# sczhou/CodeFormer

Hardware: NVIDIA H100
Metric: faces_per_sec_512x512_batch32 (higher is better)
Workload: dtype f32 (split-fp16 operands on tensor cores, fp32 accumulate)

## Files before the change

codeformer_b200/csrc/simt_kernels.cu:

```cuda
#include <cuda_fp16.h>
#include <cuda_runtime.h>

#include <atomic>
#include <math.h>
#include <stdint.h>

#include "kernels.cuh"

namespace cfb {

__device__ __forceinline__ float silu_f(float x) { return x / (1.f + expf(-x)); }
__device__ __forceinline__ float gelu_f(float x) { return 0.5f * x * (1.f + erff(x * 0.70710678118654752440f)); }
__device__ __forceinline__ float lrelu_f(float x) { return x > 0.f ? x : 0.2f * x; }

constexpr int CF_BM = 128;
constexpr int CF_BK = 16;
constexpr int CF_APITCH = CF_BM + 4;

template <int BN>
__global__ void __launch_bounds__(256) conv_f32_kernel(ConvArgs a) {
  constexpr int TN = BN / 16;
  __shared__ __align__(16) float As[2][CF_BK][CF_APITCH];
  __shared__ __align__(16) float Bs[2][CF_BK][BN];

  const int t = threadIdx.x;
  const int64_t M = (int64_t)a.N * a.Ho * a.Wo;
  const int64_t m0 = (int64_t)blockIdx.x * CF_BM;
  const int n0 = blockIdx.y * BN;
  const int taps = a.ksize * a.ksize;
  const int kchunks = a.Cin / CF_BK;
  const int nk = taps * kchunks;

  const int arow = t >> 1;
  const int akq = (t & 1) * 8;
  const int64_t am = m0 + arow;
  const bool arow_ok = am < M;
  int an = 0, aoy = 0, aox = 0;
  if (arow_ok) {
    an = (int)(am / ((int64_t)a.Ho * a.Wo));
    int rem = (int)(am - (int64_t)an * a.Ho * a.Wo);
    aoy = rem / a.Wo;
    aox = rem - aoy * a.Wo;
  }
  const float* in_n = a.in + (int64_t)an * a.H * a.W * a.Cin;
  const float* sc_n = a.in_scale ? a.in_scale + (int64_t)an * a.Cin : nullptr;
  const float* sh_n = a.in_shift ? a.in_shift + (int64_t)an * a.Cin : nullptr;

  constexpr int BV = (CF_BK * BN / 4) / 256;
  const int bcol = (BN == 128) ? (t & 31) * 4 : (t & 15) * 4;
  const int brow0 = (BN == 128) ? (t >> 5) : (t >> 4);

  float4 ra[2], rb[BV];

  auto load_global = [&](int it) {
    const int tap = it / kchunks;
    const int c0 = (it - tap * kchunks) * CF_BK;
    int r = 0, s = 0;
    if (a.ksize == 3) { r = tap / 3; s = tap - r * 3; }
    bool ok = arow_ok;
    int iy, ix;
    if (a.mode == CONV_DOWN) {
      iy = aoy * 2 + r; ix = aox * 2 + s;
      ok = ok && iy < a.H && ix < a.W;
    } else if (a.mode == CONV_UP) {
      iy = aoy + r - 1; ix = aox + s - 1;
      ok = ok && iy >= 0 && ix >= 0 && iy < 2 * a.H && ix < 2 * a.W;
      iy >>= 1; ix >>= 1;
    } else {
      const int p = a.ksize >> 1;
      iy = aoy + r - p; ix = aox + s - p;
      ok = ok && iy >= 0 && ix >= 0 && iy < a.H && ix < a.W;
    }
    if (ok) {
      const float* p = in_n + ((int64_t)iy * a.W + ix) * a.Cin + c0 + akq;
      ra[0] = __ldg(reinterpret_cast<const float4*>(p));
      ra[1] = __ldg(reinterpret_cast<const float4*>(p + 4));
      if (sc_n) {
        const float4 s0 = __ldg(reinterpret_cast<const float4*>(sc_n + c0 + akq));
        const float4 s1 = __ldg(reinterpret_cast<const float4*>(sc_n + c0 + akq + 4));
        const float4 h0 = __ldg(reinterpret_cast<const float4*>(sh_n + c0 + akq));
        const float4 h1 = __ldg(reinterpret_cast<const float4*>(sh_n + c0 + akq + 4));
        ra[0].x = fmaf(ra[0].x, s0.x, h0.x); ra[0].y = fmaf(ra[0].y, s0.y, h0.y);
        ra[0].z = fmaf(ra[0].z, s0.z, h0.z); ra[0].w = fmaf(ra[0].w, s0.w, h0.w);
        ra[1].x = fmaf(ra[1].x, s1.x, h1.x); ra[1].y = fmaf(ra[1].y, s1.y, h1.y);
        ra[1].z = fmaf(ra[1].z, s1.z, h1.z); ra[1].w = fmaf(ra[1].w, s1.w, h1.w);
      }
      if (a.in_act == IN_SILU) {
        ra[0].x = silu_f(ra[0].x); ra[0].y = silu_f(ra[0].y); ra[0].z = silu_f(ra[0].z); ra[0].w = silu_f(ra[0].w);
        ra[1].x = silu_f(ra[1].x); ra[1].y = silu_f(ra[1].y); ra[1].z = silu_f(ra[1].z); ra[1].w = silu_f(ra[1].w);
      }
    } else {
      ra[0] = make_float4(0.f, 0.f, 0.f, 0.f);
      ra[1] = ra[0];
    }
    const float* wb = a.wgt_f32 + ((int64_t)tap * a.Cin + c0) * a.Cout + n0 + bcol;
#pragma unroll
    for (int i = 0; i < BV; ++i) {
      const int kr = brow0 + i * 8;
      rb[i] = __ldg(reinterpret_cast<const float4*>(wb + (int64_t)kr * a.Cout));
    }
  };
  auto store_smem = [&](int buf) {
    As[buf][akq + 0][arow] = ra[0].x; As[buf][akq + 1][arow] = ra[0].y;
    As[buf][akq + 2][arow] = ra[0].z; As[buf][akq + 3][arow] = ra[0].w;
    As[buf][akq + 4][arow] = ra[1].x; As[buf][akq + 5][arow] = ra[1].y;
    As[buf][akq + 6][arow] = ra[1].z; As[buf][akq + 7][arow] = ra[1].w;
#pragma unroll
    for (int i = 0; i < BV; ++i) {
      const int kr = brow0 + i * 8;
      *reinterpret_cast<float4*>(&Bs[buf][kr][bcol]) = rb[i];
    }
  };

  const int ty = t >> 4, tx = t & 15;
  float acc[8][TN];
#pragma unroll
  for (int i = 0; i < 8; ++i)
#pragma unroll
    for (int j = 0; j < TN; ++j) acc[i][j] = 0.f;

  load_global(0);
  store_smem(0);
  __syncthreads();
  int buf = 0;
  for (int it = 0; it < nk; ++it) {
    if (it + 1 < nk) load_global(it + 1);
#pragma unroll
    for (int k = 0; k < CF_BK; ++k) {
      const float4 a0 = *reinterpret_cast<const float4*>(&As[buf][k][ty * 4]);
      const float4 a1 = *reinterpret_cast<const float4*>(&As[buf][k][64 + ty * 4]);
      const float av[8] = {a0.x, a0.y, a0.z, a0.w, a1.x, a1.y, a1.z, a1.w};
      float bv[TN];
      {
        const float4 b0 = *reinterpret_cast<const float4*>(&Bs[buf][k][tx * 4]);
        bv[0] = b0.x; bv[1] = b0.y; bv[2] = b0.z; bv[3] = b0.w;
        if (TN == 8) {
          const float4 b1 = *reinterpret_cast<const float4*>(&Bs[buf][k][(BN / 2) + tx * 4]);
          bv[TN - 4] = b1.x; bv[TN - 3] = b1.y; bv[TN - 2] = b1.z; bv[TN - 1] = b1.w;
        }
      }
#pragma unroll
      for (int i = 0; i < 8; ++i)
#pragma unroll
        for (int j = 0; j < TN; ++j) acc[i][j] = fmaf(av[i], bv[j], acc[i][j]);
    }
    if (it + 1 < nk) store_smem(buf ^ 1);
    __syncthreads();
    buf ^= 1;
  }

#pragma unroll
  for (int i = 0; i < 8; ++i) {
    const int64_t m = m0 + ((i < 4) ? (ty * 4 + i) : (64 + ty * 4 + (i - 4)));
    if (m >= M) continue;
#pragma unroll
    for (int h = 0; h < TN / 4; ++h) {
      const int col = n0 + h * (BN / 2) + tx * 4;
      float4 v = make_float4(acc[i][h * 4 + 0], acc[i][h * 4 + 1], acc[i][h * 4 + 2], acc[i][h * 4 + 3]);
      if (a.bias) {
        const float4 b = __ldg(reinterpret_cast<const float4*>(a.bias + col));
        v.x += b.x; v.y += b.y; v.z += b.z; v.w += b.w;
      }
      const int64_t off = m * a.Cout + col;
      if (a.residual) {
        const float4 r = __ldg(reinterpret_cast<const float4*>(a.residual + off));
        v.x += r.x; v.y += r.y; v.z += r.z; v.w += r.w;
      }
      if (a.out_act == OUT_LRELU) {
        v.x = lrelu_f(v.x); v.y = lrelu_f(v.y); v.z = lrelu_f(v.z); v.w = lrelu_f(v.w);
      } else if (a.out_act == OUT_GELU) {
        v.x = gelu_f(v.x); v.y = gelu_f(v.y); v.z = gelu_f(v.z); v.w = gelu_f(v.w);
      }
      if (a.sft_dec) {
        const float4 d = __ldg(reinterpret_cast<const float4*>(a.sft_dec + off));
        const float4 s = __ldg(reinterpret_cast<const float4*>(a.sft_scale + off));
        v.x = d.x + a.sft_w * (d.x * s.x + v.x); v.y = d.y + a.sft_w * (d.y * s.y + v.y);
        v.z = d.z + a.sft_w * (d.z * s.z + v.z); v.w = d.w + a.sft_w * (d.w * s.w + v.w);
      }
      *reinterpret_cast<float4*>(a.out + off) = v;
    }
  }
}

int conv_f32(const ConvArgs& a, cudaStream_t st) {
  CFB_REQUIRE(a.Cin % CF_BK == 0, "conv_f32: Cin must be a multiple of 16");
  CFB_REQUIRE(a.Cout % 64 == 0, "conv_f32: Cout must be a multiple of 64");
  CFB_REQUIRE(a.ksize == 1 || a.ksize == 3, "conv_f32: kernel size must be 1 or 3");
  CFB_REQUIRE(a.wgt_f32 && a.in && a.out, "conv_f32: null tensor");
  const int64_t M = (int64_t)a.N * a.Ho * a.Wo;
  if (M == 0) return 0;
  const unsigned gx = (unsigned)((M + CF_BM - 1) / CF_BM);
  if (a.Cout % 128 == 0) {
    conv_f32_kernel<128><<<dim3(gx, a.Cout / 128), 256, 0, st>>>(a);
  } else {
    conv_f32_kernel<64><<<dim3(gx, a.Cout / 64), 256, 0, st>>>(a);
  }
  CFB_LAUNCH_CHECK();
  return 0;
}

__device__ __forceinline__ float u8_to_model_input(int u) {
  const float t = (float)((double)u / 255.0);
  return __fdiv_rn(__fsub_rn(t, 0.5f), 0.5f);
}
__device__ __forceinline__ unsigned model_output_to_u8(float v) {
  float t = fminf(fmaxf(v, -1.f), 1.f);
  t = __fdiv_rn(__fadd_rn(t, 1.f), 2.f);
  return (unsigned)rintf(__fmul_rn(t, 255.f));
}

template <int COUT, bool U8>
__global__ void __launch_bounds__(256) conv_first_kernel(const float* __restrict__ x, const float* __restrict__ wgt,
                                                         const float* __restrict__ bias, float* __restrict__ out,
                                                         int N, int H, int W, float* __restrict__ gn_part) {
  __shared__ __align__(16) float ws[27 * COUT];
  __shared__ float bs[COUT];
  __shared__ float lut[U8 ? 256 : 1];
  if constexpr (U8) lut[threadIdx.x] = u8_to_model_input(threadIdx.x);
  pdl_launch_dependents();
  pdl_wait();
  for (int i = threadIdx.x; i < 27 * COUT; i += 256) ws[i] = wgt[i];
  for (int i = threadIdx.x; i < COUT; i += 256) bs[i] = bias ? bias[i] : 0.f;
  __syncthreads();
  constexpr int CPT = COUT / 4;
  const int64_t HW = (int64_t)H * W;
  const int64_t quad = (int64_t)blockIdx.x * 64 + (threadIdx.x >> 2);
  const int cg = threadIdx.x & 3;
  const int64_t pix0 = quad * 4;
  if (pix0 >= (int64_t)N * HW) return;
  const int n = (int)(pix0 / HW);
  const int rem = (int)(pix0 - (int64_t)n * HW);
  const int y = rem / W, x0 = rem - y * W;
  float acc[4][CPT];
#pragma unroll
  for (int p = 0; p < 4; ++p)
#pragma unroll
    for (int j = 0; j < CPT; ++j) acc[p][j] = bs[cg * CPT + j];
#pragma unroll
  for (int r = 0; r < 3; ++r) {
    const int iy = y + r - 1;
    const bool rowok = iy >= 0 && iy < H;
#pragma unroll
    for (int c = 0; c < 3; ++c) {
      float v[6];
      if constexpr (U8) {
        const unsigned char* rp8 = reinterpret_cast<const unsigned char*>(x) + ((int64_t)n * HW + (int64_t)iy * W) * 3 + (2 - c);
#pragma unroll
        for (int q = 0; q < 6; ++q) {
          const int ix = x0 + q - 1;
          v[q] = (rowok && ix >= 0 && ix < W) ? lut[__ldg(rp8 + ix * 3)] : 0.f;
        }
      } else {
        const float* rp = x + ((int64_t)n * 3 + c) * HW + (int64_t)iy * W;
#pragma unroll
        for (int q = 0; q < 6; ++q) {
          const int ix = x0 + q - 1;
          v[q] = (rowok && ix >= 0 && ix < W) ? __ldg(rp + ix) : 0.f;
        }
      }
#pragma unroll
      for (int s = 0; s < 3; ++s) {
        const float* wr = ws + ((r * 3 + s) * 3 + c) * COUT + cg * CPT;
#pragma unroll
        for (int j = 0; j < CPT; j += 4) {
          const float4 w4 = *reinterpret_cast<const float4*>(wr + j);
#pragma unroll
          for (int p = 0; p < 4; ++p) {
            acc[p][j] = fmaf(v[p + s], w4.x, acc[p][j]); acc[p][j + 1] = fmaf(v[p + s], w4.y, acc[p][j + 1]);
            acc[p][j + 2] = fmaf(v[p + s], w4.z, acc[p][j + 2]); acc[p][j + 3] = fmaf(v[p + s], w4.w, acc[p][j + 3]);
          }
        }
      }
    }
  }
#pragma unroll
  for (int p = 0; p < 4; ++p) {
    float* o = out + (pix0 + p) * COUT + cg * CPT;
#pragma unroll
    for (int j = 0; j < CPT; j += 4) *reinterpret_cast<float4*>(o + j) = make_float4(acc[p][j], acc[p][j + 1], acc[p][j + 2], acc[p][j + 3]);
  }
  if (gn_part != nullptr) {
    static_assert(COUT == 64, "GroupNorm partials: two channels per group");
    float gs[CPT / 2], gq[CPT / 2];
#pragma unroll
    for (int g = 0; g < CPT / 2; ++g) {
      float a = 0.f, b = 0.f;
#pragma unroll
      for (int p = 0; p < 4; ++p) {
        a += acc[p][2 * g] + acc[p][2 * g + 1];
        b += fmaf(acc[p][2 * g], acc[p][2 * g], acc[p][2 * g + 1] * acc[p][2 * g + 1]);
      }
#pragma unroll
      for (int o = 4; o < 32; o <<= 1) { a += __shfl_xor_sync(0xffffffffu, a, o); b += __shfl_xor_sync(0xffffffffu, b, o); }
      gs[g] = a; gq[g] = b;
    }
    if ((threadIdx.x & 31) < 4) {
      const int64_t slot = pix0 / 32;
      float2* dst = reinterpret_cast<float2*>(gn_part) + slot * 32 + cg * (CPT / 2);
#pragma unroll
      for (int g = 0; g < CPT / 2; ++g) dst[g] = make_float2(gs[g], gq[g]);
    }
  }
}

int conv_first(const float* x, const float* wgt, const float* bias, float* out, int N, int H, int W, int Cout,
               cudaStream_t st, float* gn_part) {
  CFB_REQUIRE(Cout == 64, "conv_first: only nf=64 is built");
  CFB_REQUIRE(W % 4 == 0, "conv_first: W must be a multiple of 4");
  const int64_t quads = (int64_t)N * H * W / 4;
  if (quads == 0) return 0;
  CFB_REQUIRE(gn_part == nullptr || ((int64_t)H * W) % 256 == 0, "conv_first: GroupNorm partials need H*W % 256 == 0");
  CFB_LAUNCH_PDL((conv_first_kernel<64, false>), dim3((unsigned)((quads + 63) / 64)), dim3(256), 0, st, x, wgt, bias, out, N, H, W, gn_part);
  return 0;
}
int conv_first_u8(const unsigned char* x_bgr_hwc, const float* wgt, const float* bias, float* out, int N, int H, int W,
                  int Cout, cudaStream_t st, float* gn_part) {
  CFB_REQUIRE(Cout == 64, "conv_first: only nf=64 is built");
  CFB_REQUIRE(W % 4 == 0, "conv_first: W must be a multiple of 4");
  const int64_t quads = (int64_t)N * H * W / 4;
  if (quads == 0) return 0;
  CFB_REQUIRE(gn_part == nullptr || ((int64_t)H * W) % 256 == 0, "conv_first: GroupNorm partials need H*W % 256 == 0");
  CFB_LAUNCH_PDL((conv_first_kernel<64, true>), dim3((unsigned)((quads + 63) / 64)), dim3(256), 0, st,
                 reinterpret_cast<const float*>(x_bgr_hwc), wgt, bias, out, N, H, W, gn_part);
  return 0;
}

template <bool U8>
__global__ void __launch_bounds__(256) conv_last_kernel(const float* __restrict__ in, const float* __restrict__ in_scale,
                                                        const float* __restrict__ in_shift, const float* __restrict__ wgt,
                                                        const float* __restrict__ bias, float* __restrict__ out, int N,
                                                        int H, int W, int Cin) {
  extern __shared__ __align__(16) float sm[];
  float* ws = sm;
  float* sc = ws + 9 * Cin * 4;
  float* sh = sc + Cin;
  const int64_t HW = (int64_t)H * W;
  const int64_t pix0 = ((int64_t)blockIdx.x * 256 + threadIdx.x) * 4;
  const int n = (int)(((int64_t)blockIdx.x * 1024) / HW);
  pdl_launch_dependents();
  pdl_wait();
  for (int i = threadIdx.x; i < 9 * Cin; i += 256) {
    ws[i * 4 + 0] = wgt[i * 3 + 0]; ws[i * 4 + 1] = wgt[i * 3 + 1]; ws[i * 4 + 2] = wgt[i * 3 + 2]; ws[i * 4 + 3] = 0.f;
  }
  for (int i = threadIdx.x; i < Cin; i += 256) {
    sc[i] = in_scale ? in_scale[(int64_t)n * Cin + i] : 1.f;
    sh[i] = in_shift ? in_shift[(int64_t)n * Cin + i] : 0.f;
  }
  __syncthreads();
  const int rem = (int)(pix0 - (int64_t)n * HW);
  const int y = rem / W, x0 = rem - y * W;
  float acc[4][3];
#pragma unroll
  for (int p = 0; p < 4; ++p) { acc[p][0] = bias ? bias[0] : 0.f; acc[p][1] = bias ? bias[1] : 0.f; acc[p][2] = bias ? bias[2] : 0.f; }
  for (int r = 0; r < 3; ++r) {
    const int iy = y + r - 1;
    if (iy < 0 || iy >= H) continue;
    const float* rowp = in + ((int64_t)n * H + iy) * W * Cin;
    for (int c = 0; c < Cin; c += 4) {
      const float4 s4 = *reinterpret_cast<const float4*>(sc + c);
      const float4 h4 = *reinterpret_cast<const float4*>(sh + c);
      float v[6][4];
#pragma unroll
      for (int q = 0; q < 6; ++q) {
        const int ix = x0 + q - 1;
        if (ix >= 0 && ix < W) {
          const float4 t = __ldg(reinterpret_cast<const float4*>(rowp + (int64_t)ix * Cin + c));
          v[q][0] = fmaf(t.x, s4.x, h4.x); v[q][1] = fmaf(t.y, s4.y, h4.y);
          v[q][2] = fmaf(t.z, s4.z, h4.z); v[q][3] = fmaf(t.w, s4.w, h4.w);
        } else {
          v[q][0] = v[q][1] = v[q][2] = v[q][3] = 0.f;
        }
      }
#pragma unroll
      for (int s = 0; s < 3; ++s) {
        const float* wt = ws + ((r * 3 + s) * Cin + c) * 4;
#pragma unroll
        for (int j = 0; j < 4; ++j) {
          const float4 w4 = *reinterpret_cast<const float4*>(wt + j * 4);
#pragma unroll
          for (int p = 0; p < 4; ++p) {
            acc[p][0] = fmaf(v[p + s][j], w4.x, acc[p][0]);
            acc[p][1] = fmaf(v[p + s][j], w4.y, acc[p][1]);
            acc[p][2] = fmaf(v[p + s][j], w4.z, acc[p][2]);
          }
        }
      }
    }
  }
  if constexpr (U8) {
    unsigned b[12];
#pragma unroll
    for (int p = 0; p < 4; ++p) {
      b[p * 3 + 0] = model_output_to_u8(acc[p][2]); b[p * 3 + 1] = model_output_to_u8(acc[p][1]); b[p * 3 + 2] = model_output_to_u8(acc[p][0]);
    }
    unsigned* o8 = reinterpret_cast<unsigned*>(reinterpret_cast<unsigned char*>(out) + ((int64_t)n * HW + rem) * 3);
#pragma unroll
    for (int k = 0; k < 3; ++k) o8[k] = b[k * 4] | (b[k * 4 + 1] << 8) | (b[k * 4 + 2] << 16) | (b[k * 4 + 3] << 24);
  } else {
    float* o = out + (int64_t)n * 3 * HW + rem;
#pragma unroll
    for (int k = 0; k < 3; ++k)
      *reinterpret_cast<float4*>(o + k * HW) = make_float4(acc[0][k], acc[1][k], acc[2][k], acc[3][k]);
  }
}

int conv_last(const float* in, const float* in_scale, const float* in_shift, const float* wgt, const float* bias,
              float* out, int N, int H, int W, int Cin, cudaStream_t st) {
  const int64_t HW = (int64_t)H * W;
  CFB_REQUIRE(HW % 1024 == 0 && W % 4 == 0 && Cin % 4 == 0, "conv_last: H*W must be a multiple of 1024, W and Cin of 4");
  if (N == 0) return 0;
  const size_t smem = (size_t)(9 * Cin * 4 + 2 * Cin) * sizeof(float);
  CFB_REQUIRE(smem <= 48 * 1024, "conv_last: Cin too large");
  CFB_LAUNCH_PDL(conv_last_kernel<false>, dim3((unsigned)(N * HW / 1024)), dim3(256), smem, st, in, in_scale, in_shift, wgt, bias, out, N, H,
                 W, Cin);
  return 0;
}
int conv_last_u8(const float* in, const float* in_scale, const float* in_shift, const float* wgt, const float* bias,
                 unsigned char* out_bgr_hwc, int N, int H, int W, int Cin, cudaStream_t st) {
  const int64_t HW = (int64_t)H * W;
  CFB_REQUIRE(HW % 1024 == 0 && W % 4 == 0 && Cin % 4 == 0, "conv_last: H*W must be a multiple of 1024, W and Cin of 4");
  if (N == 0) return 0;
  const size_t smem = (size_t)(9 * Cin * 4 + 2 * Cin) * sizeof(float);
  CFB_REQUIRE(smem <= 48 * 1024, "conv_last: Cin too large");
  CFB_LAUNCH_PDL(conv_last_kernel<true>, dim3((unsigned)(N * HW / 1024)), dim3(256), smem, st, in, in_scale, in_shift, wgt, bias,
                 reinterpret_cast<float*>(out_bgr_hwc), N, H, W, Cin);
  return 0;
}

__global__ void u8_to_input_kernel(const unsigned char* __restrict__ img, float* __restrict__ x, int64_t HW, int64_t total) {
  for (int64_t i = (int64_t)blockIdx.x * blockDim.x + threadIdx.x; i < total; i += (int64_t)gridDim.x * blockDim.x) {
    const int64_t n = i / (3 * HW);
    const int64_t r = i - n * 3 * HW;
    const int c = (int)(r / HW);
    const int64_t px = r - (int64_t)c * HW;
    x[i] = u8_to_model_input(img[(n * HW + px) * 3 + (2 - c)]);
  }
}
__global__ void output_to_u8_kernel(const float* __restrict__ x, unsigned char* __restrict__ img, int64_t HW, int64_t total) {
  for (int64_t i = (int64_t)blockIdx.x * blockDim.x + threadIdx.x; i < total; i += (int64_t)gridDim.x * blockDim.x) {
    const int64_t n = i / (3 * HW);
    const int64_t r = i - n * 3 * HW;
    const int64_t px = r / 3;
    const int k = (int)(r - px * 3);
    img[i] = (unsigned char)model_output_to_u8(x[(n * 3 + (2 - k)) * HW + px]);
  }
}
int u8_to_input(const unsigned char* img_bgr_hwc, float* x_nchw, int N, int64_t HW, cudaStream_t st) {
  const int64_t total = (int64_t)N * 3 * HW;
  if (total == 0) return 0;
  u8_to_input_kernel<<<(unsigned)((total + 255) / 256 > 148 * 16 ? 148 * 16 : (total + 255) / 256), 256, 0, st>>>(img_bgr_hwc, x_nchw, HW, total);
  CFB_LAUNCH_CHECK();
  return 0;
}
int output_to_u8(const float* x_nchw, unsigned char* img_bgr_hwc, int N, int64_t HW, cudaStream_t st) {
  const int64_t total = (int64_t)N * 3 * HW;
  if (total == 0) return 0;
  output_to_u8_kernel<<<(unsigned)((total + 255) / 256 > 148 * 16 ? 148 * 16 : (total + 255) / 256), 256, 0, st>>>(x_nchw, img_bgr_hwc, HW, total);
  CFB_LAUNCH_CHECK();
  return 0;
}

__global__ void relayout_oihw_kernel(const float* __restrict__ w, float* __restrict__ out, int Cout, int Cin, int k) {
  const int64_t total = (int64_t)Cout * Cin * k * k;
  for (int64_t i = (int64_t)blockIdx.x * blockDim.x + threadIdx.x; i < total; i += (int64_t)gridDim.x * blockDim.x) {
    const int co = (int)(i % Cout);
    const int ci = (int)((i / Cout) % Cin);
    const int tap = (int)(i / ((int64_t)Cout * Cin));
    out[i] = w[((int64_t)co * Cin + ci) * k * k + tap];
  }
}
int relayout_oihw_to_tck(const float* oihw, float* out, int Cout, int Cin, int k, cudaStream_t st) {
  const int64_t total = (int64_t)Cout * Cin * k * k;
  relayout_oihw_kernel<<<(unsigned)((total + 255) / 256 > 4096 ? 4096 : (total + 255) / 256), 256, 0, st>>>(oihw, out, Cout,
                                                                                                          Cin, k);
  CFB_LAUNCH_CHECK();
  return 0;
}

static inline int gn_chunk_pixels(int HW) { return HW < 2048 ? HW : 2048; }
size_t gn_workspace_bytes(int N, int HW, int C) {
  const int chunks = HW / gn_chunk_pixels(HW);
  return (size_t)N * chunks * 32 * 2 * sizeof(double);
}

__global__ void __launch_bounds__(256) gn_partial_kernel(const float* __restrict__ x, double* __restrict__ part, int HW,
                                                         int C, int CP, int groups) {
  __shared__ float ssum[256 * 4];
  __shared__ float ssq[256 * 4];
  __shared__ double csum[1024];
  __shared__ double csq[1024];
  const int t = threadIdx.x;
  const int C4 = C >> 2;
  const int PL = 256 / C4;
  const int c4 = t % C4, pl = t / C4;
  const int chunk = blockIdx.x, n = blockIdx.y, chunks = gridDim.x;
  const float* base = x + ((int64_t)n * HW + (int64_t)chunk * CP) * C + c4 * 4;
  float s[4] = {0.f, 0.f, 0.f, 0.f}, q[4] = {0.f, 0.f, 0.f, 0.f};
  for (int p = pl; p < CP; p += PL) {
    const float4 v = __ldg(reinterpret_cast<const float4*>(base + (int64_t)p * C));
    s[0] += v.x; s[1] += v.y; s[2] += v.z; s[3] += v.w;
    q[0] = fmaf(v.x, v.x, q[0]); q[1] = fmaf(v.y, v.y, q[1]); q[2] = fmaf(v.z, v.z, q[2]); q[3] = fmaf(v.w, v.w, q[3]);
  }
#pragma unroll
  for (int j = 0; j < 4; ++j) { ssum[pl * C + c4 * 4 + j] = s[j]; ssq[pl * C + c4 * 4 + j] = q[j]; }
  __syncthreads();
  for (int c = t; c < C; c += 256) {
    double a = 0.0, b = 0.0;
    for (int l = 0; l < PL; ++l) { a += (double)ssum[l * C + c]; b += (double)ssq[l * C + c]; }
    csum[c] = a; csq[c] = b;
  }
  __syncthreads();
  if (t < groups) {
    const int cpg = C / groups;
    double a = 0.0, b = 0.0;
    for (int c = 0; c < cpg; ++c) { a += csum[t * cpg + c]; b += csq[t * cpg + c]; }
    double* o = part + (((int64_t)n * chunks + chunk) * groups + t) * 2;
    o[0] = a; o[1] = b;
  }
}

__global__ void gn_final_kernel(const double* __restrict__ part, const float* __restrict__ gamma,
                                const float* __restrict__ beta, float* __restrict__ scale, float* __restrict__ shift,
                                int HW, int C, int chunks, int groups, float eps) {
  __shared__ double gmean[64], grstd[64];
  const int n = blockIdx.x, t = threadIdx.x;
  const int cpg = C / groups;
  if (t < groups) {
    double a = 0.0, b = 0.0;
    for (int k = 0; k < chunks; ++k) {
      const double* p = part + (((int64_t)n * chunks + k) * groups + t) * 2;
      a += p[0]; b += p[1];
    }
    const double cnt = (double)HW * cpg;
    const double mean = a / cnt;
    double var = b / cnt - mean * mean;
    if (var < 0.0) var = 0.0;
    gmean[t] = mean;
    grstd[t] = 1.0 / sqrt(var + (double)eps);
  }
  __syncthreads();
  for (int c = t; c < C; c += blockDim.x) {
    const int g = c / cpg;
    const double sc = grstd[g] * (double)gamma[c];
    scale[(int64_t)n * C + c] = (float)sc;
    shift[(int64_t)n * C + c] = (float)((double)beta[c] - gmean[g] * sc);
  }
}

int gn_coef(const float* x, const float* gamma, const float* beta, float* scale, float* shift, int N, int HW, int C,
            int groups, float eps, void* ws, cudaStream_t st) {
  CFB_REQUIRE(C % 4 == 0 && (C / 4) <= 256 && 256 % (C / 4) == 0, "gn_coef: C must be 4*divisor of 256");
  CFB_REQUIRE(groups <= 64 && C % groups == 0, "gn_coef: bad group count");
  const int CP = gn_chunk_pixels(HW);
  CFB_REQUIRE(HW % CP == 0, "gn_coef: H*W must be a multiple of the chunk size");
  if (N == 0) return 0;
  const int chunks = HW / CP;
  gn_partial_kernel<<<dim3(chunks, N), 256, 0, st>>>(x, (double*)ws, HW, C, CP, groups);
  CFB_LAUNCH_CHECK();
  gn_final_kernel<<<N, 256, 0, st>>>((const double*)ws, gamma, beta, scale, shift, HW, C, chunks, groups, eps);
  CFB_LAUNCH_CHECK();
  return 0;
}

__host__ __device__ inline int gn_final_split(int slots) {
  int g = slots / 256;
  return g < 1 ? 1 : (g > 16 ? 16 : g);
}
__global__ void __launch_bounds__(256) gn_final_f32_kernel(const float* __restrict__ part, const float* __restrict__ gamma,
                                                           const float* __restrict__ beta, float* __restrict__ scale,
                                                           float* __restrict__ shift, int HW, int C, int slots, float eps,
                                                           double* __restrict__ part2, unsigned* __restrict__ counters) {
  __shared__ double ps[8][33], pq[8][33];
  __shared__ double gmean[32], grstd[32];
  __shared__ int is_last;
  pdl_launch_dependents();
  pdl_wait();
  const int n = blockIdx.y, G = gridDim.x, blk = blockIdx.x, t = threadIdx.x;
  const int g = t & 31, stripe = t >> 5;
  const int per = (slots + G - 1) / G;
  const int lo = blk * per, hi = min(slots, lo + per);
  double a = 0.0, b = 0.0;
  const float2* base = reinterpret_cast<const float2*>(part) + (int64_t)n * slots * 32 + g;
  int k = lo + stripe;
  for (; k + 24 < hi; k += 32) {
    const float2 v0 = __ldg(base + (int64_t)k * 32), v1 = __ldg(base + (int64_t)(k + 8) * 32);
    const float2 v2 = __ldg(base + (int64_t)(k + 16) * 32), v3 = __ldg(base + (int64_t)(k + 24) * 32);
    a += ((double)v0.x + (double)v1.x) + ((double)v2.x + (double)v3.x);
    b += ((double)v0.y + (double)v1.y) + ((double)v2.y + (double)v3.y);
  }
  for (; k < hi; k += 8) {
    const float2 v = __ldg(base + (int64_t)k * 32);
    a += (double)v.x; b += (double)v.y;
  }
  ps[stripe][g] = a; pq[stripe][g] = b;
  __syncthreads();
  double sa = 0.0, sb = 0.0;
  if (t < 32) {
    for (int s = 0; s < 8; ++s) { sa += ps[s][t]; sb += pq[s][t]; }
  }
  if (G > 1) {
    if (t < 32) {
      double* dst = part2 + ((int64_t)n * G + blk) * 64;
      dst[2 * t] = sa; dst[2 * t + 1] = sb;
      __threadfence();
    }
    __syncthreads();
    if (t == 0) is_last = (atomicAdd(counters + n, 1u) == (unsigned)(G - 1));
    __syncthreads();
    if (!is_last) return;
    __threadfence();
    if (t < 32) {
      sa = 0.0; sb = 0.0;
      const double* src = part2 + (int64_t)n * G * 64;
      for (int q = 0; q < G; ++q) { sa += __ldcg(src + q * 64 + 2 * t); sb += __ldcg(src + q * 64 + 2 * t + 1); }
    }
    if (t == 0) counters[n] = 0u;
  }
  const int cpg = C / 32;
  if (t < 32) {
    const double cnt = (double)HW * cpg;
    const double mean = sa / cnt;
    double var = sb / cnt - mean * mean;
    if (var < 0.0) var = 0.0;
    gmean[t] = mean;
    grstd[t] = 1.0 / sqrt(var + (double)eps);
  }
  __syncthreads();
  for (int c = t; c < C; c += 256) {
    const int gg = c / cpg;
    const double sc = grstd[gg] * (double)gamma[c];
    scale[(int64_t)n * C + c] = (float)sc;
    shift[(int64_t)n * C + c] = (float)((double)beta[c] - gmean[gg] * sc);
  }
}
size_t gn_final_scratch_bytes(int N, int slots) {
  const int G = gn_final_split(slots);
  return G > 1 ? (size_t)N * G * 64 * sizeof(double) : 0;
}
int gn_coef_from_partials(const float* part, int slots, const float* gamma, const float* beta, float* scale, float* shift,
                          int N, int HW, int C, int groups, float eps, void* scratch, unsigned* counters, cudaStream_t st) {
  CFB_REQUIRE(groups == 32 && C % 32 == 0, "gn_coef_from_partials: 32 groups only");
  if (N == 0) return 0;
  const int G = gn_final_split(slots);
  CFB_REQUIRE(G == 1 || (scratch && counters), "gn_coef_from_partials: scratch / counters missing");
  CFB_REQUIRE(N <= 65535, "gn_coef_from_partials: batch too large");
  CFB_LAUNCH_PDL(gn_final_f32_kernel, dim3(G, N), dim3(256), 0, st, part, gamma, beta, scale, shift, HW, C, slots, eps, (double*)scratch,
                 counters);
  return 0;
}

__global__ void gn_cat_partials_kernel(const float2* __restrict__ a, const float2* __restrict__ b, float2* __restrict__ out,
                                       int64_t total) {
  pdl_launch_dependents();
  pdl_wait();
  for (int64_t i = (int64_t)blockIdx.x * blockDim.x + threadIdx.x; i < total; i += (int64_t)gridDim.x * blockDim.x) {
    const int g = (int)(i & 31);
    const int64_t slot = i >> 5;
    const float2* src = (g < 16) ? a + slot * 32 + 2 * g : b + slot * 32 + 2 * (g - 16);
    const float2 u = __ldg(src), v = __ldg(src + 1);
    out[i] = make_float2(u.x + v.x, u.y + v.y);
  }
}
int gn_cat_partials(const float* a_part, const float* b_part, float* out_part, int64_t total_slots, cudaStream_t st) {
  const int64_t total = total_slots * 32;
  if (total == 0) return 0;
  const int64_t blocks = (total + 255) / 256;
  CFB_LAUNCH_PDL(gn_cat_partials_kernel, dim3((unsigned)(blocks > 2048 ? 2048 : blocks)), dim3(256), 0, st, (const float2*)a_part,
                 (const float2*)b_part, (float2*)out_part, total);
  return 0;
}

__global__ void affine_act_kernel(const float4* __restrict__ x, const float* __restrict__ scale,
                                  const float* __restrict__ shift, float4* __restrict__ y, int64_t total4, int64_t HWC4,
                                  int C, int act) {
  for (int64_t i = (int64_t)blockIdx.x * blockDim.x + threadIdx.x; i < total4; i += (int64_t)gridDim.x * blockDim.x) {
    const int n = (int)(i / HWC4);
    const int c = (int)((i * 4) % C);
    float4 v = __ldg(x + i);
    if (scale) {
      const float4 s = __ldg(reinterpret_cast<const float4*>(scale + (int64_t)n * C + c));
      const float4 h = __ldg(reinterpret_cast<const float4*>(shift + (int64_t)n * C + c));
      v.x = fmaf(v.x, s.x, h.x); v.y = fmaf(v.y, s.y, h.y); v.z = fmaf(v.z, s.z, h.z); v.w = fmaf(v.w, s.w, h.w);
    }
    if (act == IN_SILU) { v.x = silu_f(v.x); v.y = silu_f(v.y); v.z = silu_f(v.z); v.w = silu_f(v.w); }
    y[i] = v;
  }
}
int affine_act(const float* x, const float* scale, const float* shift, float* y, int N, int HW, int C, int act,
               cudaStream_t st) {
  CFB_REQUIRE(C % 4 == 0, "affine_act: C must be a multiple of 4");
  const int64_t total4 = (int64_t)N * HW * C / 4;
  if (total4 == 0) return 0;
  const int64_t blocks = (total4 + 255) / 256;
  affine_act_kernel<<<(unsigned)(blocks > 148 * 16 ? 148 * 16 : blocks), 256, 0, st>>>(
      (const float4*)x, scale, shift, (float4*)y, total4, (int64_t)HW * C / 4, C, act);
  CFB_LAUNCH_CHECK();
  return 0;
}

__device__ __forceinline__ void split_store4(__half* __restrict__ hi, __half* __restrict__ lo, int64_t off, const float4& o);

constexpr int AT_S = 256;
constexpr int AT_QB = 32;

template <int D>
__global__ void __launch_bounds__(256) attention_kernel(const float* __restrict__ q, const float* __restrict__ k,
                                                        const float* __restrict__ v, float* __restrict__ out, int q_pitch,
                                                        int k_pitch, int v_pitch, int o_pitch, float scale,
                                                        __half* __restrict__ out_hi, __half* __restrict__ out_lo) {
  extern __shared__ __align__(16) float sm[];
  float* Qs = sm;
  float* Ks = Qs + 32 * AT_QB;
  float* P = Ks + 32 * AT_S;
  const int t = threadIdx.x;
  const int q0 = blockIdx.x * AT_QB, h = blockIdx.y, b = blockIdx.z;
  const int qg = t >> 5, kg = t & 31;
  const float* qb = q + ((int64_t)b * AT_S + q0) * q_pitch + h * D;
  const float* kb = k + ((int64_t)b * AT_S) * k_pitch + h * D;
  const float* vb = v + ((int64_t)b * AT_S) * v_pitch + h * D;

  float s[4][8];
#pragma unroll
  for (int i = 0; i < 4; ++i)
#pragma unroll
    for (int j = 0; j < 8; ++j) s[i][j] = 0.f;

  for (int d0 = 0; d0 < D; d0 += 32) {
    {
      const int qi = t >> 3, dd4 = (t & 7) * 4;
// ... 1006 lines not shown
```

Baseline: 135.6.

## Stage conv_last input halo tile in swizzled shared memory

The final 3x3 conv to RGB now stages a 4x64 pixel tile plus halo of the normalized input into shared memory, with an XOR swizzle on float4 channel groups. Each thread then computes one output pixel from shared memory instead of four pixels read straight from global memory. This removes redundant global reads across neighbouring rows and columns and folds the per-channel scale and shift into the staging pass. The cost is much more shared memory (about 150KB at Cin=128), which allows fewer resident blocks per SM, plus narrower per-pixel output stores.

```diff
diff --git a/codeformer_b200/csrc/simt_kernels.cu b/codeformer_b200/csrc/simt_kernels.cu
--- a/codeformer_b200/csrc/simt_kernels.cu
+++ b/codeformer_b200/csrc/simt_kernels.cu
@@ -325,6 +325,11 @@
   return 0;
 }
 
+constexpr int CL_TH = 4, CL_TW = 64;
+constexpr int CL_PH = CL_TH + 2, CL_PW = CL_TW + 2;
+constexpr int CL_MAX_CIN = 128;
+static size_t conv_last_smem(int Cin) { return (size_t)(9 * Cin * 4 + CL_PH * CL_PW * Cin) * sizeof(float); }
+
 template <bool U8>
 __global__ void __launch_bounds__(256) conv_last_kernel(const float* __restrict__ in, const float* __restrict__ in_scale,
                                                         const float* __restrict__ in_shift, const float* __restrict__ wgt,
@@ -332,99 +337,97 @@
                                                         int H, int W, int Cin) {
   extern __shared__ __align__(16) float sm[];
   float* ws = sm;
-  float* sc = ws + 9 * Cin * 4;
-  float* sh = sc + Cin;
-  const int64_t HW = (int64_t)H * W;
-  const int64_t pix0 = ((int64_t)blockIdx.x * 256 + threadIdx.x) * 4;
-  const int n = (int)(((int64_t)blockIdx.x * 1024) / HW);
+  float* xs = ws + 9 * Cin * 4;
+  const int Q = Cin / 4;
+  const int tiles_x = (W + CL_TW - 1) / CL_TW, tiles_y = (H + CL_TH - 1) / CL_TH;
+  const int n = (int)(blockIdx.x / (unsigned)(tiles_x * tiles_y));
+  const int trem = (int)blockIdx.x - n * tiles_x * tiles_y;
+  const int y0 = (trem / tiles_x) * CL_TH, x0 = (trem % tiles_x) * CL_TW;
   pdl_launch_dependents();
   pdl_wait();
   for (int i = threadIdx.x; i < 9 * Cin; i += 256) {
     ws[i * 4 + 0] = wgt[i * 3 + 0]; ws[i * 4 + 1] = wgt[i * 3 + 1]; ws[i * 4 + 2] = wgt[i * 3 + 2]; ws[i * 4 + 3] = 0.f;
   }
-  for (int i = threadIdx.x; i < Cin; i += 256) {
-    sc[i] = in_scale ? in_scale[(int64_t)n * Cin + i] : 1.f;
-    sh[i] = in_shift ? in_shift[(int64_t)n * Cin + i] : 0.f;
-  }
-  __syncthreads();
-  const int rem = (int)(pix0 - (int64_t)n * HW);
-  const int y = rem / W, x0 = rem - y * W;
-  float acc[4][3];
-#pragma unroll
-  for (int p = 0; p < 4; ++p) { acc[p][0] = bias ? bias[0] : 0.f; acc[p][1] = bias ? bias[1] : 0.f; acc[p][2] = bias ? bias[2] : 0.f; }
+  for (int i = threadIdx.x; i < CL_PH * CL_PW * Q; i += 256) {
+    const int q = i % Q, pix = i / Q;
+    const int pr = pix / CL_PW, pc = pix - pr * CL_PW;
+    const int iy = y0 - 1 + pr, ix = x0 - 1 + pc;
+    float4 v = make_float4(0.f, 0.f, 0.f, 0.f);
+    if (iy >= 0 && iy < H && ix >= 0 && ix < W) {
+      const float4 t = __ldg(reinterpret_cast<const float4*>(in + (((int64_t)n * H + iy) * W + ix) * Cin) + q);
+      const float4 s4 = in_scale ? __ldg(reinterpret_cast<const float4*>(in_scale + (int64_t)n * Cin) + q) : make_float4(1.f, 1.f, 1.f, 1.f);
+      const float4 h4 = in_shift ? __ldg(reinterpret_cast<const float4*>(in_shift + (int64_t)n * Cin) + q) : make_float4(0.f, 0.f, 0.f, 0.f);
+      v = make_float4(fmaf(t.x, s4.x, h4.x), fmaf(t.y, s4.y, h4.y), fmaf(t.z, s4.z, h4.z), fmaf(t.w, s4.w, h4.w));
+    }
+    reinterpret_cast<float4*>(xs)[pix * Q + (q ^ (pc & 7))] = v;
+  }
+  __syncthreads();
+  const int tr = threadIdx.x / CL_TW, tc = threadIdx.x % CL_TW;
+  const int y = y0 + tr, x = x0 + tc;
+  float acc[3];
+  acc[0] = bias ? bias[0] : 0.f; acc[1] = bias ? bias[1] : 0.f; acc[2] = bias ? bias[2] : 0.f;
   for (int r = 0; r < 3; ++r) {
     const int iy = y + r - 1;
     if (iy < 0 || iy >= H) continue;
-    const float* rowp = in + ((int64_t)n * H + iy) * W * Cin;
+    const float4* prow = reinterpret_cast<const float4*>(xs) + (tr + r) * CL_PW * Q;
     for (int c = 0; c < Cin; c += 4) {
-      const float4 s4 = *reinterpret_cast<const float4*>(sc + c);
-      const float4 h4 = *reinterpret_cast<const float4*>(sh + c);
-      float v[6][4];
-#pragma unroll
-      for (int q = 0; q < 6; ++q) {
-        const int ix = x0 + q - 1;
-        if (ix >= 0 && ix < W) {
-          const float4 t = __ldg(reinterpret_cast<const float4*>(rowp + (int64_t)ix * Cin + c));
-          v[q][0] = fmaf(t.x, s4.x, h4.x); v[q][1] = fmaf(t.y, s4.y, h4.y);
-          v[q][2] = fmaf(t.z, s4.z, h4.z); v[q][3] = fmaf(t.w, s4.w, h4.w);
-        } else {
-          v[q][0] = v[q][1] = v[q][2] = v[q][3] = 0.f;
-        }
-      }
+      float4 v[3];
+#pragma unroll
+      for (int s = 0; s < 3; ++s) v[s] = prow[(tc + s) * Q + ((c >> 2) ^ ((tc + s) & 7))];
 #pragma unroll
       for (int s = 0; s < 3; ++s) {
         const float* wt = ws + ((r * 3 + s) * Cin + c) * 4;
+        const float vj[4] = {v[s].x, v[s].y, v[s].z, v[s].w};
 #pragma unroll
         for (int j = 0; j < 4; ++j) {
           const float4 w4 = *reinterpret_cast<const float4*>(wt + j * 4);
-#pragma unroll
-          for (int p = 0; p < 4; ++p) {
-            acc[p][0] = fmaf(v[p + s][j], w4.x, acc[p][0]);
-            acc[p][1] = fmaf(v[p + s][j], w4.y, acc[p][1]);
-            acc[p][2] = fmaf(v[p + s][j], w4.z, acc[p][2]);
-          }
+          acc[0] = fmaf(vj[j], w4.x, acc[0]);
+          acc[1] = fmaf(vj[j], w4.y, acc[1]);
+          acc[2] = fmaf(vj[j], w4.z, acc[2]);
         }
       }
     }
   }
+  if (y >= H || x >= W) return;
+  const int64_t HW = (int64_t)H * W, pix = (int64_t)y * W + x;
   if constexpr (U8) {
-    unsigned b[12];
-#pragma unroll
-    for (int p = 0; p < 4; ++p) {
-      b[p * 3 + 0] = model_output_to_u8(acc[p][2]); b[p * 3 + 1] = model_output_to_u8(acc[p][1]); b[p * 3 + 2] = model_output_to_u8(acc[p][0]);
-    }
-    unsigned* o8 = reinterpret_cast<unsigned*>(reinterpret_cast<unsigned char*>(out) + ((int64_t)n * HW + rem) * 3);
-#pragma unroll
-    for (int k = 0; k < 3; ++k) o8[k] = b[k * 4] | (b[k * 4 + 1] << 8) | (b[k * 4 + 2] << 16) | (b[k * 4 + 3] << 24);
+    unsigned char* o8 = reinterpret_cast<unsigned char*>(out) + ((int64_t)n * HW + pix) * 3;
+    o8[0] = (unsigned char)model_output_to_u8(acc[2]); o8[1] = (unsigned char)model_output_to_u8(acc[1]);
+    o8[2] = (unsigned char)model_output_to_u8(acc[0]);
   } else {
-    float* o = out + (int64_t)n * 3 * HW + rem;
-#pragma unroll
-    for (int k = 0; k < 3; ++k)
-      *reinterpret_cast<float4*>(o + k * HW) = make_float4(acc[0][k], acc[1][k], acc[2][k], acc[3][k]);
-  }
+    float* o = out + (int64_t)n * 3 * HW + pix;
+#pragma unroll
+    for (int k = 0; k < 3; ++k) o[k * HW] = acc[k];
+  }
+}
+
+template <bool U8>
+static int launch_conv_last(const float* in, const float* in_scale, const float* in_shift, const float* wgt, const float* bias,
+                            float* out, int N, int H, int W, int Cin, cudaStream_t st) {
+  CFB_REQUIRE(Cin % 32 == 0 && Cin <= CL_MAX_CIN, "conv_last: Cin must be a multiple of 32 and at most 128");
+  if (N == 0 || H == 0 || W == 0) return 0;
+  static std::atomic<uint64_t> attr_done{0};
+  int dev = 0;
+  CFB_CUDA(cudaGetDevice(&dev));
+  const uint64_t bit = 1ull << (dev & 63);
+  if (!(attr_done.load(std::memory_order_acquire) & bit)) {
+    CFB_CUDA(cudaFuncSetAttribute(conv_last_kernel<U8>, cudaFuncAttributeMaxDynamicSharedMemorySize, (int)conv_last_smem(CL_MAX_CIN)));
+    attr_done.fetch_or(bit, std::memory_order_release);
+  }
+  const int64_t tiles = (int64_t)N * ((H + CL_TH - 1) / CL_TH) * ((W + CL_TW - 1) / CL_TW);
+  CFB_REQUIRE(tiles <= 0x7fffffffLL, "conv_last: too many tiles");
+  CFB_LAUNCH_PDL(conv_last_kernel<U8>, dim3((unsigned)tiles), dim3(256), conv_last_smem(Cin), st, in, in_scale, in_shift, wgt, bias,
+                 out, N, H, W, Cin);
+  return 0;
 }
 
 int conv_last(const float* in, const float* in_scale, const float* in_shift, const float* wgt, const float* bias,
               float* out, int N, int H, int W, int Cin, cudaStream_t st) {
-  const int64_t HW = (int64_t)H * W;
-  CFB_REQUIRE(HW % 1024 == 0 && W % 4 == 0 && Cin % 4 == 0, "conv_last: H*W must be a multiple of 1024, W and Cin of 4");
-  if (N == 0) return 0;
-  const size_t smem = (size_t)(9 * Cin * 4 + 2 * Cin) * sizeof(float);
-  CFB_REQUIRE(smem <= 48 * 1024, "conv_last: Cin too large");
-  CFB_LAUNCH_PDL(conv_last_kernel<false>, dim3((unsigned)(N * HW / 1024)), dim3(256), smem, st, in, in_scale, in_shift, wgt, bias, out, N, H,
-                 W, Cin);
-  return 0;
+  return launch_conv_last<false>(in, in_scale, in_shift, wgt, bias, out, N, H, W, Cin, st);
 }
 int conv_last_u8(const float* in, const float* in_scale, const float* in_shift, const float* wgt, const float* bias,
                  unsigned char* out_bgr_hwc, int N, int H, int W, int Cin, cudaStream_t st) {
-  const int64_t HW = (int64_t)H * W;
-  CFB_REQUIRE(HW % 1024 == 0 && W % 4 == 0 && Cin % 4 == 0, "conv_last: H*W must be a multiple of 1024, W and Cin of 4");
-  if (N == 0) return 0;
-  const size_t smem = (size_t)(9 * Cin * 4 + 2 * Cin) * sizeof(float);
-  CFB_REQUIRE(smem <= 48 * 1024, "conv_last: Cin too large");
-  CFB_LAUNCH_PDL(conv_last_kernel<true>, dim3((unsigned)(N * HW / 1024)), dim3(256), smem, st, in, in_scale, in_shift, wgt, bias,
-                 reinterpret_cast<float*>(out_bgr_hwc), N, H, W, Cin);
-  return 0;
+  return launch_conv_last<true>(in, in_scale, in_shift, wgt, bias, reinterpret_cast<float*>(out_bgr_hwc), N, H, W, Cin, st);
 }
 
 __global__ void u8_to_input_kernel(const unsigned char* __restrict__ img, float* __restrict__ x, int64_t HW, int64_t total) {
```

Measured after the change: 140.2, median of 6. 3.4% higher.
